# ComputationalPhysiology/oasisx

Hardware: AMD Instinct MI355X
Metric: time-steps/sec, 3D Taylor-Green 128^3 P2-P1 (with pressure-CG SpMV GB/s in roofline) (higher is better)
Workload: dtype f64

## Files before the change

### include/oasisx_hip.h

```cpp
#ifndef OASISX_HIP_H
#define OASISX_HIP_H

#include <stddef.h>
#include <stdint.h>

#ifdef __cplusplus
extern "C" {
#endif

#define OX_KV 2
#define OX_ROW_BLOCK_WAVES 8
#define OX_ROW_BLOCK_LDS (134 * 1024)
#define OX_SLICE 64

#define OX_CONVERGED_RTOL 2
#define OX_CONVERGED_ATOL 3
#define OX_CONVERGED_ITS 4
#define OX_DIVERGED_ITS (-3)
#define OX_DIVERGED_DTOL (-4)
#define OX_DIVERGED_BREAKDOWN (-5)
#define OX_DIVERGED_NANORINF (-9)

#define OX_KSP_CG 1
#define OX_KSP_BCGS 2
// ... 143 lines not shown
int ox_rect_view(const ox_rect *rect, ox_rect_info *view);
int ox_rect_destroy(ox_rect *rect);
int ox_value_dictionary(const double *vals, int64_t n_slots, int ncomp, void *codes, double *dict, int *n_dict,
                        void *stream);
int ox_pair_stream_size(const ox_sell *A, const int32_t *row_len, int64_t *ps_ptr, int64_t *n_codes, void *stream);
int ox_window_retile(const ox_sell *A, const int64_t *wt_ptr, const void *src, int elem_bytes, void *dst, void *stream);
int ox_pair_stream_fill(const ox_sell *A, const int32_t *row_len, int64_t *ps_ptr, uint32_t *ps_code,
                        int32_t *ps_base, int64_t *n_wide, void *stream);
int ox_malloc(size_t bytes, void **out);
int ox_free(void *p);
int ox_memset(void *p, int value, size_t bytes, void *stream);
int ox_synchronize(void *stream);

int ox_version(void);
const char *ox_last_error(void);
int ox_sell_kv(void);
int ox_device_info(int *n_cu, char *name, int name_len);

int ox_spmv(const ox_sell *A, const double *x, double *y, int ncomp, const ox_dist *dist,
            void *stream);

int ox_sell_compress_cols(const ox_sell *A, uint16_t *cols16, int32_t *cbase, int64_t *n_compressed,
                          void *stream);

int ox_spmv_multi(int v2s, int gdim, const ox_sell *A, const double *x, const double *base, double scale,
                  double *y, const ox_dist *dist, void *stream);
int ox_assemble_rect(int family, int row_degree, int col_degree, const ox_cells *cells, const ox_adj *adj,
                     const uint8_t *adj_pos, int pw, const ox_sell *A, void *stream);

int ox_axpby(int64_t n, double a, const double *x, double b, const double *y, double *z,
             void *stream);
int ox_dot(int64_t n_rows, int ncomp, const double *x, const double *y, double *out_host,
           const ox_dist *dist, void *stream);

int ox_set_bc(double *b, const int32_t *dofs, const double *g, int64_t n, int ncomp, int comp,
              void *stream);

int ox_scatter_add(double *b, const int32_t *rows, const double *y, int64_t n, int ncomp, int comp,
                   double scale, void *stream);

int ox_zero_rows(const ox_sell *A, const int32_t *rows, int64_t n, double diag, void *stream);
int ox_zero_rows_au(const ox_sell *A, const int32_t *rows, int64_t n, double diag, double *au,
                    const double *u1, int ncomp, void *stream);
int ox_zero_rows_cols(const ox_sell *A, const uint8_t *is_bc, double diag, void *stream);

int ox_assemble_matrix(int kind, int degree, const ox_cells *cells, const int32_t *cell_dofs,
                       const ox_adj *adj, const uint8_t *adj_pos, int pw, const ox_sell *A,
                       int n_bins, const int64_t *bin_ptr_host, const int32_t *bin_slices,
                       const int32_t *bin_width_host, void *stream);
int ox_assemble_weights(int degree, const ox_cells *cells, const ox_adj *adj, int64_t n_rows,
                        double *w, void *stream);
int ox_assemble_load_vector(const ox_cells *cells, const ox_adj *adj, int64_t n_rows, int n_d, int n_q,
                            const double *wphi, const double *fq, double *b, void *stream);

int ox_assemble_first(int degree, const ox_cells *cells, const int32_t *cell_dofs,
                      const ox_adj *adj, const uint8_t *adj_pos, int pw, const ox_sell *A,
                      const ox_sell *M, const ox_sell *K, const double *uab,
                      const double *u1, const double *b0, double *b_first, double dt, double nu,
                      int n_bins, const int64_t *bin_ptr_host, const int32_t *bin_slices,
                      const int32_t *bin_width_host, void *stream);

int ox_assemble_first_au(int degree, const ox_cells *cells, const int32_t *cell_dofs,
                         const ox_adj *adj, const uint8_t *adj_pos, int pw, const ox_sell *A,
                         const ox_sell *M, const ox_sell *K, const double *uab,
                         const double *u1, const double *b0, double *b_first, double dt, double nu,
                         int n_bins, const int64_t *bin_ptr_host, const int32_t *bin_slices,
// ... 154 lines not shown
```

### oasisx_amd/_lib.py

```python
from __future__ import annotations

import ctypes as C
import os

_HERE = os.path.dirname(os.path.abspath(__file__))
LIB_PATH = os.environ.get("OX_LIB_PATH") or os.path.join(_HERE, "liboasisx_hip.so")

KSP_CG, KSP_BCGS, KSP_CG_SINGLE, KSP_BCGS_MERGED, KSP_CG_MERGED = 1, 2, 3, 4, 5
KSP_CG_MG = 6
MG_MAX_DEGREE = 8
ROW_BLOCK_WAVES, ROW_BLOCK_LDS = 8, 134 * 1024
CONVERGED_RTOL, CONVERGED_ATOL, CONVERGED_ITS = 2, 3, 4
DIVERGED_ITS, DIVERGED_DTOL, DIVERGED_BREAKDOWN, DIVERGED_NANORINF = -3, -4, -5, -9


class OasisxHipError(RuntimeError):
    pass


class ox_sell(C.Structure):
    _fields_ = [
        ("n_rows", C.c_int64),
        ("n_cols", C.c_int64),
        ("n_slices", C.c_int32),
# ... 175 lines not shown

SIGNATURES = {
    "ox_version": (_I, []),
    "ox_last_error": (C.c_char_p, []),
    "ox_sell_kv": (_I, []),
    "ox_device_info": (_I, [C.POINTER(_I), C.c_char_p, _I]),
    "ox_mesh_create": (_I, [_P, _L, _P, _L, _I, _I, _I, C.POINTER(_P)]),
    "ox_mesh_view": (_I, [_P, C.POINTER(ox_mesh_info)]),
    "ox_mesh_destroy": (_I, [_P]),
    "ox_space_create": (_I, [_P, _I, _I, C.POINTER(_P)]),
    "ox_space_create_ordered": (_I, [_P, _I, _I, _I, C.POINTER(_P)]),
    "ox_mesh_create_sub": (_I, [_P, _L, _P, _L, _I, _I, C.POINTER(_D), C.POINTER(_D), _I, _I, _L, C.POINTER(_P)]),
    "ox_space_create_part": (_I, [_P, _I, _I, _P, _L, _I, _L, C.POINTER(_P)]),
    "ox_space_view": (_I, [_P, C.POINTER(ox_space_info)]),
    "ox_space_windows": (_I, [_P, C.POINTER(ox_window_info)]),
    "ox_space_windows_split": (_I, [_P, _I, C.POINTER(ox_window_info)]),
    "ox_space_destroy": (_I, [_P]),
    "ox_rect_create": (_I, [_P, _P, C.POINTER(_P)]),
    "ox_rect_view": (_I, [_P, C.POINTER(ox_rect_info)]),
    "ox_rect_destroy": (_I, [_P]),
    "ox_value_dictionary": (_I, [_P, _L, _I, _P, _P, C.POINTER(_I), _P]),
    "ox_pair_stream_size": (_I, [C.POINTER(ox_sell), _P, _P, C.POINTER(_L), _P]),
    "ox_pair_stream_fill": (_I, [C.POINTER(ox_sell), _P, _P, _P, _P, C.POINTER(_L), _P]),
    "ox_malloc": (_I, [C.c_size_t, C.POINTER(_P)]),
    "ox_free": (_I, [_P]),
    "ox_memset": (_I, [_P, _I, C.c_size_t, _P]),
    "ox_synchronize": (_I, [_P]),
    "ox_spmv": (_I, [C.POINTER(ox_sell), _P, _P, _I, _P, _P]),
    "ox_sell_compress_cols": (_I, [C.POINTER(ox_sell), _P, _P, C.POINTER(_L), _P]),
    "ox_spmv_multi": (_I, [_I, _I, C.POINTER(ox_sell), _P, _P, _D, _P, _P, _P]),
    "ox_assemble_rect": (_I, [_I, _I, _I, C.POINTER(ox_cells), C.POINTER(ox_adj), _P, _I, C.POINTER(ox_sell), _P]),
    "ox_axpby": (_I, [_L, _D, _P, _D, _P, _P, _P]),
    "ox_dot": (_I, [_L, _I, _P, _P, C.POINTER(_D), _P, _P]),
    "ox_set_bc": (_I, [_P, _P, _P, _L, _I, _I, _P]),
    "ox_scatter_add": (_I, [_P, _P, _P, _L, _I, _I, _D, _P]),
    "ox_zero_rows": (_I, [C.POINTER(ox_sell), _P, _L, _D, _P]),
    "ox_zero_rows_au": (_I, [C.POINTER(ox_sell), _P, _L, _D, _P, _P, _I, _P]),
    "ox_zero_rows_cols": (_I, [C.POINTER(ox_sell), _P, _D, _P]),
    "ox_assemble_matrix": (_I, [_I, _I, C.POINTER(ox_cells), _P, C.POINTER(ox_adj), _P, _I,
                                C.POINTER(ox_sell), _I, C.POINTER(_L), _P, C.POINTER(C.c_int32), _P]),
    "ox_assemble_weights": (_I, [_I, C.POINTER(ox_cells), C.POINTER(ox_adj), _L, _P, _P]),
    "ox_assemble_load_vector": (_I, [C.POINTER(ox_cells), C.POINTER(ox_adj), _L, _I, _I, _P, _P, _P, _P]),
    "ox_assemble_first": (_I, [_I, C.POINTER(ox_cells), _P, C.POINTER(ox_adj), _P, _I,
                               C.POINTER(ox_sell), C.POINTER(ox_sell), C.POINTER(ox_sell), _P, _P, _P, _P, _D,
                               _D, _I, C.POINTER(_L), _P, C.POINTER(C.c_int32), _P]),
    "ox_assemble_first_au": (_I, [_I, C.POINTER(ox_cells), _P, C.POINTER(ox_adj), _P, _I,
                                  C.POINTER(ox_sell), C.POINTER(ox_sell), C.POINTER(ox_sell), _P, _P, _P, _P, _D,
                                  _D, _I, C.POINTER(_L), _P, C.POINTER(C.c_int32), _P, _P]),
    "ox_assemble_matrix_blocks": (_I, [_I, _I, C.POINTER(ox_cells), _P, C.POINTER(ox_adj), _P, _I, C.POINTER(ox_sell), _I, _P,
                                       _L, _P]),
    "ox_assemble_first_blocks": (_I, [_I, C.POINTER(ox_cells), _P, C.POINTER(ox_adj), _P, _I,
                                      C.POINTER(ox_sell), C.POINTER(ox_sell), C.POINTER(ox_sell), _P, _P, _P, _P, _D,
                                      _D, _I, _P, _L, _P, _P]),
    "ox_assemble_grad_vector": (_I, [_I, _I, _I, C.POINTER(ox_cells), _P, C.POINTER(ox_adj), _L, _P,
                                     _P, _D, _P, _P]),
    "ox_assemble_div_vector": (_I, [_I, _I, C.POINTER(ox_cells), _P, C.POINTER(ox_adj), _L, _P, _D,
                                    _P, _P]),
    "ox_dg1_grad_rhs": (_I, [_I, C.POINTER(ox_cells), _P, _P, _P, _P]),
    "ox_dg1_mass": (_I, [_I, C.POINTER(ox_cells), _I, _P, _P, _P]),
    "ox_jacobi_setup": (_I, [C.POINTER(ox_sell), _P, _P]),
    "ox_ksp_work_bytes": (C.c_size_t, [_L, _L, _I, _I]),
    "ox_ksp_solve": (_I, [_I, C.POINTER(ox_sell), _P, _P, _P, _I, _D, _D, _I, _I, _I, _I, _P,
                          C.c_size_t, C.POINTER(ox_ksp_result), _P, _P]),
    "ox_ksp_solve_ax0": (_I, [_I, C.POINTER(ox_sell), _P, _P, _P, _I, _D, _D, _I, _I, _I, _I, _P,
                              C.c_size_t, C.POINTER(ox_ksp_result), _P, _P, _P]),
    "ox_ksp_solve_dc": (_I, [_I, C.POINTER(ox_sell), _P, _P, _P, _I, _D, _D, _I, _I, _I, _I, _P,
# ... 102 lines not shown
```

### oasisx_amd/csrc/ox_ksp.hip

```cpp
#include "ox_kernels.h"
#include "ox_ksp_dev.h"
#include "ox_p2p.h"
#include <type_traits>

struct KspPart2 {
  const double *partial;
  int nparts, nv;
};

__device__ __forceinline__ void ksp_gather2(const double *__restrict__ partial, int nparts, int nv, const KspPart2 &B,
                                            double (&v)[OX_MAX_NV]) {
  ox_gather_partials(partial, nparts, nv, v);
  if (B.nv > 0) {
    double w[OX_MAX_NV];
    ox_gather_partials(B.partial, B.nparts, B.nv, w);
#pragma unroll
    for (int i = 0; i < OX_MAX_NV; ++i)
#pragma unroll
      for (int j = 0; j < OX_MAX_NV; ++j)
        if (j == i - nv && j < B.nv) v[i] = w[j];
  }
}


// ... 654 lines not shown
    }
  });
  ksp_store_partial<2 * NC>(s, red, partial);
}

template <int NC>
__global__ __launch_bounds__(256) void k_bcgs_init(int64_t n, const double *__restrict__ b,
                                                   double *x, const double *q,
                                                   const double *__restrict__ dinv, double *vr,
                                                   double *vrhat, double *vp, double *vv, int guess,
                                                   double *partial) {
  __shared__ double red[4 * 2 * NC];
  double s[2 * NC];
#pragma unroll
  for (int i = 0; i < 2 * NC; ++i) s[i] = 0.0;
  ox_flat_pairs<NC>(n, [&](int64_t e, int ca, int64_t ra, int cb, int64_t rb, bool two) {
    const double2 bb = ox_ld2(b, e, two);
    double2 r = bb;
    if (guess) {
      const double2 qq = ox_ld2(q, e, two);
      r.x -= qq.x;
      r.y -= qq.y;
    } else {
      double2 z;
      z.x = z.y = 0.0;
      ox_st2(x, e, z, two);
    }
    const double d0 = dinv[ra], d1 = two ? dinv[rb] : 0.0;
    r.x *= d0;
    r.y *= d1;
    const double db0 = d0 * bb.x, db1 = d1 * bb.y;
    ox_st2(vr, e, r, two);
    ox_st2(vrhat, e, r, two);
    ox_st2(vp, e, r, two);
    ox_acc<NC>(s, 0, ca, r.x, r.x);
    ox_acc<NC>(s, NC, ca, db0, db0);
    if (two) {
      ox_acc<NC>(s, 0, cb, r.y, r.y);
      ox_acc<NC>(s, NC, cb, db1, db1);
    }
  });
  ksp_store_partial<2 * NC>(s, red, partial);
}

template <int NC>
__global__ __launch_bounds__(256) void k_bcgs_p(int64_t n, const KspState *S, int c0,
                                                const double *__restrict__ vr, double *vp,
                                                const double *__restrict__ vv, double *vrhat) {
  if (S->done) return;
  double beta[NC], omega[NC], reseed[NC];
  bool any = false;
#pragma unroll
  for (int c = 0; c < NC; ++c) {
    beta[c] = S->beta[c0 + c];
    omega[c] = S->omega[c0 + c];
    reseed[c] = S->restart[c0 + c] ? 1.0 : 0.0;
    any = any || S->restart[c0 + c];
  }
  ox_flat_pairs<NC>(n, [&](int64_t e, int ca, int64_t, int cb, int64_t, bool two) {
    const double2 r = ox_ld2(vr, e, two), v = ox_ld2(vv, e, two);
    double2 p = ox_ld2(vp, e, two);
    const bool ra = ox_sel<NC>(reseed, ca) != 0.0, rb = ox_sel<NC>(reseed, cb) != 0.0;
    p.x = ra ? r.x : fma(ox_sel<NC>(beta, ca), fma(-ox_sel<NC>(omega, ca), v.x, p.x), r.x);
    p.y = rb ? r.y : fma(ox_sel<NC>(beta, cb), fma(-ox_sel<NC>(omega, cb), v.y, p.y), r.y);
    ox_st2(vp, e, p, two);
    if (any) {
      double2 h = ox_ld2(vrhat, e, two);
      h.x = ra ? r.x : h.x;
      h.y = rb ? r.y : h.y;
      ox_st2(vrhat, e, h, two);
    }
  });
}

template <int NC>
__global__ __launch_bounds__(256) void k_bcgs_s(int64_t n, const KspState *S, int c0,
                                                const double *__restrict__ vr,
                                                const double *__restrict__ vv, double *vs) {
  if (S->done) return;
  double alpha[NC];
#pragma unroll
  for (int c = 0; c < NC; ++c) alpha[c] = S->alpha[c0 + c];
  ox_flat_pairs<NC>(n, [&](int64_t e, int ca, int64_t, int cb, int64_t, bool two) {
    const double2 r = ox_ld2(vr, e, two), v = ox_ld2(vv, e, two);
    double2 s;
    s.x = fma(-ox_sel<NC>(alpha, ca), v.x, r.x);
    s.y = fma(-ox_sel<NC>(alpha, cb), v.y, r.y);
    ox_st2(vs, e, s, two);
  });
}

template <int NC>
__global__ __launch_bounds__(256) void k_bcgs_x(int64_t n, const KspState *S, int c0, double *x, double *vr,
                                                const double *__restrict__ vrhat,
// ... 165 lines not shown
    if (B.nv > 0 && (int64_t)B.nparts * B.nv >= OX_PRERED_MIN) {
      const int g = ksp_prered_rows(B.nparts);
      hipLaunchKernelGGL(k_prereduce, dim3(g), dim3(256), 0, st, B.partial, B.nparts, B.nv, scr);
      B.partial = scr;
      B.nparts = g;
    }
  }
  const int nmax = nparts > B.nparts ? nparts : B.nparts;
  if (!dist) {
    hipLaunchKernelGGL((k_ksp_scalar<PH>), dim3(1), dim3(ox_red_threads(nmax)), 0, st, S, partial, nparts, nv, P, B);
    OX_LAUNCH_CHECK();
    return 0;
  }
  if (ox_prof_on) ox_prof_start(OX_TAG_SYNC_POINT, st, nv + B.nv);
  if (dist->p2p && dist->nranks <= 64) {
    int threads = ox_red_threads(nmax);
    if (threads < ox_p2p_ar_threads(dist->nranks)) threads = ox_p2p_ar_threads(dist->nranks);
    hipLaunchKernelGGL((k_ksp_scalar_p2p<PH>), dim3(1), dim3(threads), 0, st, S, partial, nparts, nv, P,
                       ox_p2p_next_allreduce(dist), B);
    if (ox_prof_on) ox_prof_stop(st);
    OX_LAUNCH_CHECK();
    return 0;
  }
  hipLaunchKernelGGL((k_ksp_reduce<PH>), dim3(1), dim3(ox_red_threads(nmax)), 0, st, partial, nparts, nv, B, sums);
  OX_LAUNCH_CHECK();
  nv += B.nv;
  if (ox_allreduce_impl(dist, sums, nv, st)) return -1;
  hipLaunchKernelGGL((k_ksp_logic<PH>), dim3(1), dim3(64), 0, st, S, sums, P);
  if (ox_prof_on) ox_prof_stop(st);
  OX_LAUNCH_CHECK();
  return 0;
}

__global__ __launch_bounds__(256) void k_extract_col(int64_t n, const double *__restrict__ src, int nc,
                                                     int c, double *__restrict__ dst) {
  const int64_t stride = (int64_t)gridDim.x * 256;
  for (int64_t i = (int64_t)blockIdx.x * 256 + threadIdx.x; i < n; i += stride) dst[i] = src[i * nc + c];
}
__global__ __launch_bounds__(256) void k_insert_col(int64_t n, const double *__restrict__ src, int nc,
                                                    int c, double *__restrict__ dst) {
  const int64_t stride = (int64_t)gridDim.x * 256;
  for (int64_t i = (int64_t)blockIdx.x * 256 + threadIdx.x; i < n; i += stride) dst[i * nc + c] = src[i];
}

struct KspVecs {
  double *x, *r, *z, *p, *q;
  double *rhat, *v, *s, *t;
  double *u, *w;
};

struct KspCtx {
  const ox_sell *A;
  const double *dinv;
  KspDinv D;
  KspState *S, *S2;
  double *sums, *partial, *partial2;
  const ox_dist *dist;
  hipStream_t st;
  int nb, nbs;
  int fold;
};

#define KSP_SYNC(PH, partial, nparts, nv)                                                       \
  do {                                                                                          \
    if (ksp_sync_point<PH>(C.S, partial, nparts, nv, C.sums, P, C.dist, C.st)) return -1;       \
  } while (0)

static int ksp_fold_blocks_default() {
  static int dflt = -1;
  if (dflt < 0) {
// ... 239 lines not shown
  for (int k = 0; k < count; ++k) {
    ox_spmv_set_epilogue_dinv(C.D.code, C.D.dict);
    const int rc = ox_spmv_dist(C.A, V.p, V.q, NC, OX_EPI_CG_M2, C.dinv, nullptr, C.partial, done, C.dist, C.st);
    ox_spmv_set_epilogue_dinv(nullptr, nullptr);
    if (rc) return -1;
    KspParams Q = ksp_last_point(P, k, count);
    Q.first = (first && k == 0) ? 1 : 0;
    if (ksp_sync_point<PH_CGM_IT>(C.S, C.partial, C.nbs, 2 * NC, C.sums, Q, C.dist, C.st,
                                  Q.first ? KspPart2{nullptr, 0, 0} : KspPart2{C.partial2, C.nb, 3 * NC}))
      return -1;
    hipLaunchKernelGGL((k_cgm_update<NC>), dim3(C.nb), dim3(256), 0, C.st, n, C.S, P.c0, V.x, V.r, V.q, C.D, V.p, C.partial2);
    OX_LAUNCH_CHECK();
  }
  return 0;
}

template <int NC>
static int cgs_iterations(const KspCtx &C, const KspVecs &V, const KspParams &P, int count) {
  const int64_t n = C.A->n_rows;
  const int *done = &C.S->done;
  for (int k = 0; k < count; ++k) {
    hipLaunchKernelGGL((k_cgs_update<NC>), dim3(C.nb), dim3(256), 0, C.st, n, C.S, P.c0, V.x, V.r, V.u, V.p, V.s, V.w,
                       C.dinv, C.partial);
    OX_LAUNCH_CHECK();
    if (ox_spmv_dist(C.A, V.u, V.w, NC, OX_EPI_DOT, nullptr, nullptr, C.partial2, done, C.dist, C.st)) return -1;
    if (ksp_sync_point<PH_CGS_IT>(C.S, C.partial, C.nb, 2 * NC, C.sums, ksp_last_point(P, k, count), C.dist, C.st,
                                  KspPart2{C.partial2, C.nbs, NC}))
      return -1;
  }
  return 0;
}

template <int NC>
static int bcgs_iterations(const KspCtx &C, const KspVecs &V, const KspParams &P, int count, bool first) {
  const int64_t n = C.A->n_rows;
  const int *done = &C.S->done;
  for (int k = 0; k < count; ++k) {
    if (!(first && k == 0)) {
      hipLaunchKernelGGL((k_bcgs_p<NC>), dim3(C.nb), dim3(256), 0, C.st, n, C.S, P.c0, V.r, V.p, V.v, V.rhat);
      OX_LAUNCH_CHECK();
    }
    if (ox_spmv_dist(C.A, V.p, V.v, NC, OX_EPI_BCGS_V, C.dinv, V.rhat, C.partial, done, C.dist, C.st)) return -1;
    KSP_SYNC(PH_BCGS_1, C.partial, C.nbs, NC);
    hipLaunchKernelGGL((k_bcgs_s<NC>), dim3(C.nb), dim3(256), 0, C.st, n, C.S, P.c0, V.r, V.v, V.s);
    OX_LAUNCH_CHECK();
    if (ox_spmv_dist(C.A, V.s, V.t, NC, OX_EPI_BCGS_T, C.dinv, nullptr, C.partial, done, C.dist, C.st)) return -1;
    KSP_SYNC(PH_BCGS_2, C.partial, C.nbs, 2 * NC);
    hipLaunchKernelGGL((k_bcgs_x<NC>), dim3(C.nb), dim3(256), 0, C.st, n, C.S, P.c0, V.x, V.r, V.rhat, V.p, V.s,
                       V.t, C.partial, 0);
    OX_LAUNCH_CHECK();
    if (ksp_sync_point<PH_BCGS_3>(C.S, C.partial, C.nb, 2 * NC, C.sums, ksp_last_point(P, k, count), C.dist, C.st)) return -1;
  }
  return 0;
}

template <int NC>
static int bcgsm_iterations(const KspCtx &C, const KspVecs &V, const KspParams &P, int count, bool first) {
  const int64_t n = C.A->n_rows;
  const int *done = &C.S->done;
  (void)first;
  for (int k = 0; k < count; ++k) {
    if (ox_spmv_dist(C.A, V.p, V.v, NC, OX_EPI_BCGS_V, C.dinv, V.rhat, C.partial, done, C.dist, C.st)) return -1;
    if (ksp_sync_point<PH_BCGS_1>(C.S, C.partial, C.nbs, NC, C.sums, P, C.dist, C.st)) return -1;
    hipLaunchKernelGGL((k_bcgs_s<NC>), dim3(C.nb), dim3(256), 0, C.st, n, C.S, P.c0, V.r, V.v, V.s);
    OX_LAUNCH_CHECK();
    if (ox_spmv_dist(C.A, V.s, V.t, NC, OX_EPI_BCGS_T5, C.dinv, V.rhat, C.partial, done, C.dist, C.st)) return -1;
    if (ksp_sync_point<PH_BCGSM_B>(C.S, C.partial, C.nbs, 5 * NC, C.sums, ksp_last_point(P, k, count), C.dist, C.st)) return -1;
    hipLaunchKernelGGL((k_bcgs_xp<NC>), dim3(C.nb), dim3(256), 0, C.st, n, C.S, P.c0, V.x, V.r, V.rhat, V.p, V.s, V.t, V.v, 0);
    OX_LAUNCH_CHECK();
  }
  return 0;
}
template <int NC>
static int bcgsm_finish(const KspCtx &C, const KspVecs &V, const KspParams &P) {
  hipLaunchKernelGGL((k_bcgs_xp<NC>), dim3(C.nb), dim3(256), 0, C.st, C.A->n_rows, C.S, P.c0, V.x, V.r, V.rhat, V.p, V.s, V.t,
                     V.v, 1);
  OX_LAUNCH_CHECK();
  return 0;
}

static int ksp_read_state(const KspCtx &C) {
  OX_HIP(hipMemcpyAsync(g_state_host, C.S, sizeof(KspState), hipMemcpyDeviceToHost, C.st));
  OX_HIP(hipStreamSynchronize(C.st));
  return C.dist ? ox_dist_status(C.dist) : 0;
// ... 62 lines not shown
  double *vec[6];
  for (int i = 0; i < L.nvec; ++i) vec[i] = reinterpret_cast<double *>(work + L.vec0 + L.vec_stride * i);
  if (!g_state_host) OX_HIP(hipHostMalloc(&g_state_host, 3 * sizeof(KspState)));
  const bool cg = ksp_type == OX_KSP_CG, cgs = ksp_type == OX_KSP_CG_SINGLE, bm = ksp_type == OX_KSP_BCGS_MERGED;
  const bool cgm = ksp_type == OX_KSP_CG_MERGED;
  KspVecs V{};
  V.x = x;
  if (cgs) {
    V.r = vec[0], V.u = vec[1], V.p = vec[2], V.s = vec[3], V.w = vec[4];
    if (guess && !ax0) {
      if (ox_spmv_dist(A, x, V.w, NC, OX_EPI_NONE, nullptr, nullptr, nullptr, nullptr, dist, st)) return -1;
    }
    hipLaunchKernelGGL((k_cgs_init<NC>), dim3(C.nb), dim3(256), 0, st, n, b, x, (guess && ax0) ? ax0 : V.w, dinv, V.r, V.u,
                       V.p, V.s, guess, C.partial);
    OX_LAUNCH_CHECK();
    if (ox_spmv_dist(A, V.u, V.w, NC, OX_EPI_DOT, nullptr, nullptr, C.partial2, nullptr, dist, st)) return -1;
    if (ksp_sync_point<PH_CGS_INIT>(C.S, C.partial, C.nb, 3 * NC, C.sums, P, dist, st, KspPart2{C.partial2, C.nbs, NC}))
      return -1;
  } else if (cg || cgm) {
    V.r = vec[0], V.p = vec[1], V.q = vec[2];
    if (guess && !ax0) {
      if (ox_spmv_dist(A, x, V.q, NC, OX_EPI_NONE, nullptr, nullptr, nullptr, nullptr, dist, st)) return -1;
    }
    hipLaunchKernelGGL((k_cg_init<NC>), dim3(C.nb), dim3(256), 0, st, n, b, x, (guess && ax0) ? ax0 : V.q, dinv, V.r,
                       V.p, guess, C.partial);
    OX_LAUNCH_CHECK();
    KSP_SYNC(PH_CG_INIT, C.partial, C.nb, 3 * NC);
  } else {
    V.r = vec[0], V.rhat = vec[1], V.p = vec[2], V.v = vec[3], V.s = vec[4], V.t = vec[5];
    if (guess && !ax0) {
      if (ox_spmv_dist(A, x, V.t, NC, OX_EPI_NONE, nullptr, nullptr, nullptr, nullptr, dist, st)) return -1;
    }
    hipLaunchKernelGGL((k_bcgs_init<NC>), dim3(C.nb), dim3(256), 0, st, n, b, x, (guess && ax0) ? ax0 : V.t, dinv, V.r,
                       V.rhat, V.p, V.v, guess, C.partial);
    OX_LAUNCH_CHECK();
    KSP_SYNC(PH_BCGS_INIT, C.partial, C.nb, 2 * NC);
  }
  bool bm_first = true;
  auto iterate = [&](auto nc_tag, const KspVecs &W, const KspParams &Q) -> int {
    constexpr int N_ = decltype(nc_tag)::value;
    const bool first = bm_first;
    bm_first = false;
    return cgs ? cgs_iterations<N_>(C, W, Q, check_every)
           : cgm ? cgm_iterations<N_>(C, W, Q, check_every, first)
               : (cg ? cg_iterations<N_>(C, W, Q, check_every)
                     : (bm ? bcgsm_iterations<N_>(C, W, Q, check_every, first) : bcgs_iterations<N_>(C, W, Q, check_every, first)));
  };
  auto batch_of = [&](int every) { return every > 8 ? 8 : every; };
  int it = 0;
  bool tail_done = false;
  for (;;) {
    tail_done = false;
    if (NC == 1 && run_ahead) {
      const int bsz = batch_of(check_every);
      auto it1 = [&](int count) -> int {
        const bool first = bm_first;
        bm_first = false;
        return cgs ? cgs_iterations<1>(C, V, P, count)
               : cgm ? cgm_iterations<1>(C, V, P, count, first)
                   : (cg ? cg_iterations<1>(C, V, P, count)
                         : (bm ? bcgsm_iterations<1>(C, V, P, count, first) : bcgs_iterations<1>(C, V, P, count, first)));
      };
      if (ksp_run_ahead(C, it1, bsz, it, P.max_it)) return -1;
    }
    for (; !(NC == 1 && run_ahead) && it <= P.max_it; it += check_every) {
      if (iterate(std::integral_constant<int, NC>{}, V, P)) return -1;
      if (ksp_read_state(C)) return -1;
      if (g_state_host->done) break;
      if (NC > 1) {
        int live = -1, nlive = 0;
        for (int c = 0; c < NC; ++c)
          if (g_state_host->active[c]) live = c, ++nlive;
        if (nlive == 1) {
          double *cv[8];
          for (int i = 0; i < 8; ++i) cv[i] = reinterpret_cast<double *>(work + L.narrow0 + L.narrow_stride * i);
          KspVecs W{};
          double *src[8] = {V.x, V.r, V.z, V.p, V.q, V.rhat, V.v, nullptr};
          double **dst[8] = {&W.x, &W.r, &W.z, &W.p, &W.q, &W.rhat, &W.v, nullptr};
          if (cg) src[2] = nullptr;
          if (cgs) {
            src[2] = V.u, dst[2] = &W.u;
            src[4] = V.s, dst[4] = &W.s;
            src[5] = V.w, dst[5] = &W.w;
            src[6] = nullptr;
          }
          for (int i = 0; i < 7; ++i) {
            *dst[i] = cv[i];
            if (!src[i]) continue;
            hipLaunchKernelGGL(k_extract_col, dim3(C.nb), dim3(256), 0, st, n, src[i], NC, live, cv[i]);
            OX_LAUNCH_CHECK();
          }
          if (!cgs) {
            W.s = cv[2];
            W.t = cv[4];
          }
          KspParams P1 = P;
          P1.nc = 1;
          P1.c0 = live;
          if (run_ahead) {
            const int bsz = batch_of(check_every);
            auto it1 = [&](int count) -> int {
              return cgs ? cgs_iterations<1>(C, W, P1, count)
                         : (cg ? cg_iterations<1>(C, W, P1, count)
                               : (bm ? bcgsm_iterations<1>(C, W, P1, count, false) : bcgs_iterations<1>(C, W, P1, count, false)));
            };
            it += check_every;
            if (ksp_run_ahead(C, it1, bsz, it, P.max_it)) return -1;
          } else {
            for (it += check_every; it <= P.max_it; it += check_every) {
              if (iterate(std::integral_constant<int, 1>{}, W, P1)) return -1;
              if (ksp_read_state(C)) return -1;
              if (g_state_host->done) break;
            }
          }
          if (cg) {
            hipLaunchKernelGGL((k_cg_update2<1>), dim3(C.nb), dim3(256), 0, st, n, C.S, P1.c0, W.x, W.r, C.D, W.p, 1);
            OX_LAUNCH_CHECK();
          }
          if (bm && g_state_host->its[live] > 0) {
            if (bcgsm_finish<1>(C, W, P1)) return -1;
            hipLaunchKernelGGL(k_insert_col, dim3(C.nb), dim3(256), 0, st, n, W.r, NC, live, V.r);
            OX_LAUNCH_CHECK();
          }
          tail_done = true;
          hipLaunchKernelGGL(k_insert_col, dim3(C.nb), dim3(256), 0, st, n, W.x, NC, live, x);
          OX_LAUNCH_CHECK();
          break;
        }
      }
    }
    if (!g_state_host->done) OX_FAIL("ox_ksp_solve: device state never reported completion");
    if (!bm) break;
    bool any = false;
    for (int c = 0; c < NC; ++c) any = any || g_state_host->its[c] > 0;
    if (!any) break;
    if (!tail_done && bcgsm_finish<NC>(C, V, P)) return -1;
    bool retest = false;
    for (int c = 0; c < NC; ++c)
      retest = retest || g_state_host->reason[c] == OX_CONVERGED_RTOL || g_state_host->reason[c] == OX_CONVERGED_ATOL;
    if (!retest) break;
    hipLaunchKernelGGL((k_rr<NC>), dim3(C.nb), dim3(256), 0, st, n, V.r, C.partial);
    OX_LAUNCH_CHECK();
    KSP_SYNC(PH_BCGSM_FIN, C.partial, C.nb, NC);
    if (ksp_read_state(C)) return -1;
    if (g_state_host->done) break;
    hipLaunchKernelGGL((k_bcgs_p<NC>), dim3(C.nb), dim3(256), 0, st, n, C.S, P.c0, V.r, V.p, V.v, V.rhat);
    OX_LAUNCH_CHECK();
    it = 0;
    for (int c = 0; c < NC; ++c) it = g_state_host->its[c] > it ? g_state_host->its[c] : it;
  }
  if (cg && !tail_done) {
    hipLaunchKernelGGL((k_cg_update2<NC>), dim3(C.nb), dim3(256), 0, st, n, C.S, P.c0, V.x, V.r, C.D, V.p, 1);
    OX_LAUNCH_CHECK();
  }
  for (int c = 0; c < NC; ++c) {
    result->reason[c] = g_state_host->reason[c];
    result->its[c] = g_state_host->its[c];
    result->rnorm[c] = g_state_host->rn[c];
    result->bnorm[c] = g_state_host->bn[c];
    result->resumed[c] = bm ? g_state_host->nresume[c] : 0;
  }
  return 0;
}

__global__ __launch_bounds__(256) void k_mgcg_init(int64_t n, const double *__restrict__ b, double *x,
                                                   const double *__restrict__ q, double *r, int guess) {
  OX_ROW_LOOP {
    if (guess) {
      r[row] = b[row] - q[row];
    } else {
      r[row] = b[row];
      x[row] = 0.0;
    }
  }
}
template <bool INIT>
__global__ __launch_bounds__(256) void k_mgcg_dots(int64_t n, const KspState *S, const double *__restrict__ r,
                                                   const double *__restrict__ z, const double *__restrict__ zb, double *p,
                                                   double *partial) {
// ... 211 lines not shown
                               size_t work_bytes, ox_ksp_result *result, const ox_dist *dist, void *stream,
                               const double *ax0, const uint8_t *dinv_code, const double *dinv_dict, int n_dinv_dict) {
  ox_ksp_options o;
  ox_ksp_options_default(&o);
  o.rtol = rtol;
  o.atol = atol;
  o.max_it = max_it;
  o.nonzero_guess = nonzero_guess;
  o.check_every = check_every;
  o.max_restarts = max_restarts;
  o.ax0 = ax0;
  o.dinv_code = dinv_code;
  o.dinv_dict = dinv_dict;
  o.n_dinv_dict = n_dinv_dict;
  return ox_ksp_solve_opt(ksp_type, A, dinv, b, x, ncomp, &o, work, work_bytes, result, dist, stream);
}

extern "C" int ox_ksp_solve_ax0(int ksp_type, const ox_sell *A, const double *dinv, const double *b,
                                double *x, int ncomp, double rtol, double atol, int max_it,
                                int nonzero_guess, int check_every, int max_restarts, void *work,
                                size_t work_bytes, ox_ksp_result *result, const ox_dist *dist, void *stream,
                                const double *ax0) {
  return ox_ksp_solve_dc(ksp_type, A, dinv, b, x, ncomp, rtol, atol, max_it, nonzero_guess, check_every, max_restarts,
                         work, work_bytes, result, dist, stream, ax0, nullptr, nullptr, 0);
}

extern "C" int ox_ksp_solve(int ksp_type, const ox_sell *A, const double *dinv, const double *b,
                            double *x, int ncomp, double rtol, double atol, int max_it,
                            int nonzero_guess, int check_every, int max_restarts, void *work,
                            size_t work_bytes, ox_ksp_result *result, const ox_dist *dist, void *stream) {
  return ox_ksp_solve_dc(ksp_type, A, dinv, b, x, ncomp, rtol, atol, max_it, nonzero_guess, check_every, max_restarts,
                         work, work_bytes, result, dist, stream, nullptr, nullptr, nullptr, 0);
}
```

### oasisx_amd/fracstep.py

```python
from __future__ import annotations

import ctypes as C
import logging

import numpy as np
import torch

from . import _lib
from .fem import FieldStorage, Function, FunctionSpace, VectorFunctionSpace, cell_geometry
from .ksp import KSPSolver
from .la import MultiSellMatrix, SellMatrix

__all__ = ["FractionalStep_AB_CN"]


def _degree(element):
    if isinstance(element, FunctionSpace):
        return element.degree
    fam = str(element[0]).lower()
    if fam not in ("lagrange", "p", "cg"):
        raise ValueError(f"unsupported element family {element[0]!r}")
    return int(element[1])


# ... 303 lines not shown
        if self._scalar_groups:
            self._A_pre_bc = True
            try:
                self.scalar_assemble(dt, nu)
            finally:
                self._A_pre_bc = False
        for bcp in self._bcs_p:
            bcp.update_bc()
            bcp.add_surface_terms(self._BFIRST)
        for bcu in self._bcs_u[0]:
            self._A.zero_rows(bcu._rows_dev, 1.0, self._B3.ptr() if want_au else None,
                              self._U1.rptr() if want_au else None, self._gdim)
        self._AU1_valid = want_au

    @_phase
    def velocity_tentative_assemble(self):
        Vi, Q = self._Vi[0][0], self._Q
        if not self._low_memory:
            self._p_vdxi_Mat.mult(False, self._PS.ptr(), self._BFIRST.ptr(), 1.0, self._RHS1.ptr())
            return
        _lib.check(self._lib.ox_assemble_grad_vector(0, Vi.degree, Q.degree, C.byref(self._cells),
                                                     _lib.ptr(Q.cell_dofs), C.byref(self._adj_u), Vi.n_owned,
                                                     self._PS.ptr(), self._BFIRST.ptr(), 1.0, self._RHS1.ptr(),
                                                     _lib.current_stream()), "ox_assemble_grad_vector")

    @_phase
    def velocity_tentative_solve(self):
        lib, st = self._lib, _lib.current_stream()
        gdim = self._gdim
        for i in range(gdim):
            for bc in self._bcs_u[i]:
                bc.apply(self._rhs1[i].x)
        n = self._n_u * gdim
        _lib.check(lib.ox_axpby(n, 1.0, self._U.rptr(), 0.0, None, self._WRK.ptr(), st), "ox_axpby")
        ax0 = None
        if getattr(self, "_AU1_valid", False):
            self._AU1_valid = False
            same = getattr(self, "_u_is_u1", None) == (self._U.generation, self._U1.generation)
            if self._part is not None and getattr(self._comm, "size", 1) > 1:
                same = self._comm.allreduce(0.0 if same else 1.0, op="max") == 0.0
            if same:
                ax0 = self._B3
            elif not getattr(self, "_shortcut_note", False):
                self._shortcut_note = True
                logging.getLogger("oasisx").info(
                    "tentative solve: u was handed out writable since the last step (FieldStorage.dev() / ptr() / host()): "
                    "the A u1 product of assemble_first is not reused; read-only access goes through rdev() / rptr() / rhost()")
        self._u_is_u1 = None
        errors = np.asarray(self._solver_u.solve_block(self._RHS1, self._U, ax0=ax0), dtype=np.int32)
        _lib.check(lib.ox_axpby(n, 1.0, self._WRK.ptr(), -1.0, self._U.ptr(), self._WRK.ptr(), st), "ox_axpby")
        out = (C.c_double * 4)()
        _lib.check(lib.ox_dot(self._no_u, gdim, self._WRK.ptr(), self._WRK.ptr(), out, self._du, st), "ox_dot")
        diff = float(sum(np.sqrt(out[i]) for i in range(gdim)))
        return diff, errors

    @_phase
    def pressure_assemble(self, dt: float):
        Vi, Q = self._Vi[0][0], self._Q
        if not self._low_memory:
            self._divu_Mat.mult(True, self._U.ptr(), None, -1.0 / float(dt), self._B2.ptr())
        else:
            _lib.check(self._lib.ox_assemble_div_vector(Q.degree, Vi.degree, C.byref(self._cells),
                                                        _lib.ptr(Vi.cell_dofs), C.byref(self._adj_q), Q.n_owned,
                                                        self._U.ptr(), -1.0 / float(dt), self._B2.ptr(),
                                                        _lib.current_stream()), "ox_assemble_div_vector")
        for bcp in self._bcs_p:
            bcp.apply_homogeneous(self._b2.x)

    @_phase
    def pressure_solve(self, nu: float | None = None, rotational: bool = False):
        lib, st = self._lib, _lib.current_stream()
        logger = logging.getLogger("oasisx")
        nq, nqo = self._n_q, self._no_q
        if len(self._bcs_p) == 0:
            if "ksp_error_if_not_converged" not in self._solver_p._options:
                self._solver_p.updateOptions({"ksp_error_if_not_converged": 1})
            _lib.check(lib.ox_remove_mean(nqo, nqo, self._B2.ptr(), None, float(self._Q.num_dofs_global),
                                          self._dq, st), "ox_remove_mean")
        converged = self._solver_p.solve_block(self._B2, self._DP)[0]
        if len(self._bcs_p) == 0:
            logger.debug("Making sure that mean of phi is 0 with lack of pressure conditions")
            _lib.check(lib.ox_remove_mean(nqo, nq, self._DP.ptr(), _lib.ptr(self._wQ), self._vol, self._dq, st),
                       "ox_remove_mean")
        if self._projector_p is not None:
            if nu is None:
# ... 104 lines not shown
```

Before: 12.22.

## Fuse velocity diff norm, skip redundant copies in BiCGStab and column extraction

Replaces the copy-then-axpby-then-dot sequence in the tentative velocity solve with a fused difference-norm kernel, and skips the initial copy of u entirely when u still equals u1. In BiCGStab the first-iteration search direction is read from rhat instead of writing a separate p vector, using a small state machine. The per-vector column extraction launches are batched into a single kernel. The aim is to cut memory traffic and launch count, at the cost of more complex state tracking for p across the batched and split paths.

```diff
diff --git a/include/oasisx_hip.h b/include/oasisx_hip.h
--- a/include/oasisx_hip.h
+++ b/include/oasisx_hip.h
@@ -199,6 +199,8 @@
              void *stream);
 int ox_dot(int64_t n_rows, int ncomp, const double *x, const double *y, double *out_host,
            const ox_dist *dist, void *stream);
+int ox_diff_norm2(int64_t n_rows, int ncomp, const double *x, const double *y, double *out_host,
+                  const ox_dist *dist, void *stream);
 
 int ox_set_bc(double *b, const int32_t *dofs, const double *g, int64_t n, int ncomp, int comp,
               void *stream);
diff --git a/oasisx_amd/_lib.py b/oasisx_amd/_lib.py
--- a/oasisx_amd/_lib.py
+++ b/oasisx_amd/_lib.py
@@ -231,6 +231,7 @@
     "ox_assemble_rect": (_I, [_I, _I, _I, C.POINTER(ox_cells), C.POINTER(ox_adj), _P, _I, C.POINTER(ox_sell), _P]),
     "ox_axpby": (_I, [_L, _D, _P, _D, _P, _P, _P]),
     "ox_dot": (_I, [_L, _I, _P, _P, C.POINTER(_D), _P, _P]),
+    "ox_diff_norm2": (_I, [_L, _I, _P, _P, C.POINTER(_D), _P, _P]),
     "ox_set_bc": (_I, [_P, _P, _P, _L, _I, _I, _P]),
     "ox_scatter_add": (_I, [_P, _P, _P, _L, _I, _I, _D, _P]),
     "ox_zero_rows": (_I, [C.POINTER(ox_sell), _P, _L, _D, _P]),
diff --git a/oasisx_amd/csrc/ox_ksp.hip b/oasisx_amd/csrc/ox_ksp.hip
--- a/oasisx_amd/csrc/ox_ksp.hip
+++ b/oasisx_amd/csrc/ox_ksp.hip
@@ -710,7 +710,7 @@
     const double db0 = d0 * bb.x, db1 = d1 * bb.y;
     ox_st2(vr, e, r, two);
     ox_st2(vrhat, e, r, two);
-    ox_st2(vp, e, r, two);
+    if (vp) ox_st2(vp, e, r, two);
     ox_acc<NC>(s, 0, ca, r.x, r.x);
     ox_acc<NC>(s, NC, ca, db0, db0);
     if (two) {
@@ -724,7 +724,7 @@
 template <int NC>
 __global__ __launch_bounds__(256) void k_bcgs_p(int64_t n, const KspState *S, int c0,
                                                 const double *__restrict__ vr, double *vp,
-                                                const double *__restrict__ vv, double *vrhat) {
+                                                const double *__restrict__ vv, double *vrhat, const double *vpin) {
   if (S->done) return;
   double beta[NC], omega[NC], reseed[NC];
   bool any = false;
@@ -737,7 +737,7 @@
   }
   ox_flat_pairs<NC>(n, [&](int64_t e, int ca, int64_t, int cb, int64_t, bool two) {
     const double2 r = ox_ld2(vr, e, two), v = ox_ld2(vv, e, two);
-    double2 p = ox_ld2(vp, e, two);
+    double2 p = ox_ld2(vpin, e, two);
     const bool ra = ox_sel<NC>(reseed, ca) != 0.0, rb = ox_sel<NC>(reseed, cb) != 0.0;
     p.x = ra ? r.x : fma(ox_sel<NC>(beta, ca), fma(-ox_sel<NC>(omega, ca), v.x, p.x), r.x);
     p.y = rb ? r.y : fma(ox_sel<NC>(beta, cb), fma(-ox_sel<NC>(omega, cb), v.y, p.y), r.y);
@@ -969,10 +969,22 @@
   return 0;
 }
 
-__global__ __launch_bounds__(256) void k_extract_col(int64_t n, const double *__restrict__ src, int nc,
-                                                     int c, double *__restrict__ dst) {
+struct KspExtract {
+  const double *src[6];
+  double *dst[6];
+  int count;
+};
+__global__ __launch_bounds__(256) void k_extract_cols(int64_t n, KspExtract E, int nc, int c) {
   const int64_t stride = (int64_t)gridDim.x * 256;
-  for (int64_t i = (int64_t)blockIdx.x * 256 + threadIdx.x; i < n; i += stride) dst[i] = src[i * nc + c];
+  for (int64_t i = (int64_t)blockIdx.x * 256 + threadIdx.x; i < n; i += stride) {
+    double v[6];
+#pragma unroll
+    for (int k = 0; k < 6; ++k)
+      if (k < E.count) v[k] = E.src[k][i * nc + c];
+#pragma unroll
+    for (int k = 0; k < 6; ++k)
+      if (k < E.count) E.dst[k][i] = v[k];
+  }
 }
 __global__ __launch_bounds__(256) void k_insert_col(int64_t n, const double *__restrict__ src, int nc,
                                                     int c, double *__restrict__ dst) {
@@ -1278,24 +1290,28 @@
 }
 
 template <int NC>
-static int bcgs_iterations(const KspCtx &C, const KspVecs &V, const KspParams &P, int count, bool first) {
+static int bcgs_iterations(const KspCtx &C, const KspVecs &V, const KspParams &P, int count, int &pstate) {
   const int64_t n = C.A->n_rows;
   const int *done = &C.S->done;
   for (int k = 0; k < count; ++k) {
-    if (!(first && k == 0)) {
-      hipLaunchKernelGGL((k_bcgs_p<NC>), dim3(C.nb), dim3(256), 0, C.st, n, C.S, P.c0, V.r, V.p, V.v, V.rhat);
+    if (pstate == 1 || pstate == 2) {
+      hipLaunchKernelGGL((k_bcgs_p<NC>), dim3(C.nb), dim3(256), 0, C.st, n, C.S, P.c0, V.r, V.p, V.v, V.rhat,
+                         pstate == 1 ? V.rhat : V.p);
       OX_LAUNCH_CHECK();
-    }
-    if (ox_spmv_dist(C.A, V.p, V.v, NC, OX_EPI_BCGS_V, C.dinv, V.rhat, C.partial, done, C.dist, C.st)) return -1;
+      pstate = 2;
+    }
+    const double *p = pstate == 0 ? V.rhat : V.p;
+    if (ox_spmv_dist(C.A, const_cast<double *>(p), V.v, NC, OX_EPI_BCGS_V, C.dinv, V.rhat, C.partial, done, C.dist, C.st)) return -1;
     KSP_SYNC(PH_BCGS_1, C.partial, C.nbs, NC);
     hipLaunchKernelGGL((k_bcgs_s<NC>), dim3(C.nb), dim3(256), 0, C.st, n, C.S, P.c0, V.r, V.v, V.s);
     OX_LAUNCH_CHECK();
     if (ox_spmv_dist(C.A, V.s, V.t, NC, OX_EPI_BCGS_T, C.dinv, nullptr, C.partial, done, C.dist, C.st)) return -1;
     KSP_SYNC(PH_BCGS_2, C.partial, C.nbs, 2 * NC);
-    hipLaunchKernelGGL((k_bcgs_x<NC>), dim3(C.nb), dim3(256), 0, C.st, n, C.S, P.c0, V.x, V.r, V.rhat, V.p, V.s,
+    hipLaunchKernelGGL((k_bcgs_x<NC>), dim3(C.nb), dim3(256), 0, C.st, n, C.S, P.c0, V.x, V.r, V.rhat, p, V.s,
                        V.t, C.partial, 0);
     OX_LAUNCH_CHECK();
     if (ksp_sync_point<PH_BCGS_3>(C.S, C.partial, C.nb, 2 * NC, C.sums, ksp_last_point(P, k, count), C.dist, C.st)) return -1;
+    pstate = pstate == 0 ? 1 : 2;
   }
   return 0;
 }
@@ -1424,11 +1440,12 @@
       if (ox_spmv_dist(A, x, V.t, NC, OX_EPI_NONE, nullptr, nullptr, nullptr, nullptr, dist, st)) return -1;
     }
     hipLaunchKernelGGL((k_bcgs_init<NC>), dim3(C.nb), dim3(256), 0, st, n, b, x, (guess && ax0) ? ax0 : V.t, dinv, V.r,
-                       V.rhat, V.p, V.v, guess, C.partial);
+                       V.rhat, (bm || dist) ? V.p : nullptr, V.v, guess, C.partial);
     OX_LAUNCH_CHECK();
     KSP_SYNC(PH_BCGS_INIT, C.partial, C.nb, 2 * NC);
   }
   bool bm_first = true;
+  int bcgs_p_state = dist ? 3 : 0;
   auto iterate = [&](auto nc_tag, const KspVecs &W, const KspParams &Q) -> int {
     constexpr int N_ = decltype(nc_tag)::value;
     const bool first = bm_first;
@@ -1436,7 +1453,7 @@
     return cgs ? cgs_iterations<N_>(C, W, Q, check_every)
            : cgm ? cgm_iterations<N_>(C, W, Q, check_every, first)
                : (cg ? cg_iterations<N_>(C, W, Q, check_every)
-                     : (bm ? bcgsm_iterations<N_>(C, W, Q, check_every, first) : bcgs_iterations<N_>(C, W, Q, check_every, first)));
+                     : (bm ? bcgsm_iterations<N_>(C, W, Q, check_every, first) : bcgs_iterations<N_>(C, W, Q, check_every, bcgs_p_state)));
   };
   auto batch_of = [&](int every) { return every > 8 ? 8 : every; };
   int it = 0;
@@ -1451,7 +1468,7 @@
         return cgs ? cgs_iterations<1>(C, V, P, count)
                : cgm ? cgm_iterations<1>(C, V, P, count, first)
                    : (cg ? cg_iterations<1>(C, V, P, count)
-                         : (bm ? bcgsm_iterations<1>(C, V, P, count, first) : bcgs_iterations<1>(C, V, P, count, first)));
+                         : (bm ? bcgsm_iterations<1>(C, V, P, count, first) : bcgs_iterations<1>(C, V, P, count, bcgs_p_state)));
       };
       if (ksp_run_ahead(C, it1, bsz, it, P.max_it)) return -1;
     }
@@ -1476,12 +1493,18 @@
             src[5] = V.w, dst[5] = &W.w;
             src[6] = nullptr;
           }
+          if (cg) src[4] = nullptr;
+          if (bcgs_p_state < 2 && !cg && !cgs && !bm) src[3] = V.rhat;
+          KspExtract E{};
           for (int i = 0; i < 7; ++i) {
             *dst[i] = cv[i];
             if (!src[i]) continue;
-            hipLaunchKernelGGL(k_extract_col, dim3(C.nb), dim3(256), 0, st, n, src[i], NC, live, cv[i]);
-            OX_LAUNCH_CHECK();
+            E.src[E.count] = src[i], E.dst[E.count] = cv[i];
+            ++E.count;
           }
+          hipLaunchKernelGGL(k_extract_cols, dim3(C.nb), dim3(256), 0, st, n, E, NC, live);
+          OX_LAUNCH_CHECK();
+          bcgs_p_state = 2;
           if (!cgs) {
             W.s = cv[2];
             W.t = cv[4];
@@ -1494,7 +1517,7 @@
             auto it1 = [&](int count) -> int {
               return cgs ? cgs_iterations<1>(C, W, P1, count)
                          : (cg ? cg_iterations<1>(C, W, P1, count)
-                               : (bm ? bcgsm_iterations<1>(C, W, P1, count, false) : bcgs_iterations<1>(C, W, P1, count, false)));
+                               : (bm ? bcgsm_iterations<1>(C, W, P1, count, false) : bcgs_iterations<1>(C, W, P1, count, bcgs_p_state)));
             };
             it += check_every;
             if (ksp_run_ahead(C, it1, bsz, it, P.max_it)) return -1;
@@ -1536,7 +1559,7 @@
     KSP_SYNC(PH_BCGSM_FIN, C.partial, C.nb, NC);
     if (ksp_read_state(C)) return -1;
     if (g_state_host->done) break;
-    hipLaunchKernelGGL((k_bcgs_p<NC>), dim3(C.nb), dim3(256), 0, st, n, C.S, P.c0, V.r, V.p, V.v, V.rhat);
+    hipLaunchKernelGGL((k_bcgs_p<NC>), dim3(C.nb), dim3(256), 0, st, n, C.S, P.c0, V.r, V.p, V.v, V.rhat, V.p);
     OX_LAUNCH_CHECK();
     it = 0;
     for (int c = 0; c < NC; ++c) it = g_state_host->its[c] > it ? g_state_host->its[c] : it;
@@ -1814,3 +1837,53 @@
   return ox_ksp_solve_dc(ksp_type, A, dinv, b, x, ncomp, rtol, atol, max_it, nonzero_guess, check_every, max_restarts,
                          work, work_bytes, result, dist, stream, nullptr, nullptr, nullptr, 0);
 }
+
+template <int NC>
+__global__ __launch_bounds__(256) void k_diff_norm2(int64_t n_rows, const double *__restrict__ x, const double *__restrict__ y,
+                                                    double *__restrict__ partial) {
+  __shared__ double red[4 * NC];
+  double s[NC];
+#pragma unroll
+  for (int c = 0; c < NC; ++c) s[c] = 0.0;
+  const int64_t stride = (int64_t)gridDim.x * 256;
+  for (int64_t r = (int64_t)blockIdx.x * 256 + threadIdx.x; r < n_rows; r += stride) {
+#pragma unroll
+    for (int c = 0; c < NC; ++c) {
+      const double d = x[r * NC + c] - y[r * NC + c];
+      s[c] = fma(d, d, s[c]);
+    }
+  }
+  ox_block_sum_256<NC>(s, red);
+  if (threadIdx.x == 0) {
+#pragma unroll
+    for (int c = 0; c < NC; ++c) partial[(size_t)blockIdx.x * NC + c] = s[c];
+  }
+}
+
+static thread_local double *g_diff_scratch = nullptr;
+static thread_local double *g_diff_scratch_host = nullptr;
+
+extern "C" int ox_diff_norm2(int64_t n_rows, int ncomp, const double *x, const double *y, double *out_host,
+                             const ox_dist *dist, void *stream) {
+  if (ncomp < 1 || ncomp > OX_MAXC) OX_FAIL("ox_diff_norm2: ncomp=%d", ncomp);
+  if (!x || !y || !out_host) OX_FAIL("ox_diff_norm2: null argument");
+  if (!g_diff_scratch) {
+    OX_HIP(hipMalloc(&g_diff_scratch, sizeof(double) * (OX_VEC_MAX_BLOCKS * 4 + 16)));
+    OX_HIP(hipHostMalloc(&g_diff_scratch_host, sizeof(double) * 16));
+  }
+  hipStream_t st = ox_stream(stream);
+  const int nblk = ox_vec_blocks(n_rows > 0 ? n_rows : 1);
+  double *partial = g_diff_scratch, *sums = g_diff_scratch + OX_VEC_MAX_BLOCKS * 4;
+  switch (ncomp) {
+    case 1: hipLaunchKernelGGL(k_diff_norm2<1>, dim3(nblk), dim3(256), 0, st, n_rows, x, y, partial); break;
+    case 2: hipLaunchKernelGGL(k_diff_norm2<2>, dim3(nblk), dim3(256), 0, st, n_rows, x, y, partial); break;
+    default: hipLaunchKernelGGL(k_diff_norm2<3>, dim3(nblk), dim3(256), 0, st, n_rows, x, y, partial); break;
+  }
+  OX_LAUNCH_CHECK();
+  if (ox_reduce_partials(partial, nblk, ncomp, sums, st)) return -1;
+  if (dist && ox_allreduce_impl(dist, sums, ncomp, st)) return -1;
+  OX_HIP(hipMemcpyAsync(g_diff_scratch_host, sums, sizeof(double) * ncomp, hipMemcpyDeviceToHost, st));
+  OX_HIP(hipStreamSynchronize(st));
+  for (int c = 0; c < ncomp; ++c) out_host[c] = g_diff_scratch_host[c];
+  return 0;
+}
diff --git a/oasisx_amd/fracstep.py b/oasisx_amd/fracstep.py
--- a/oasisx_amd/fracstep.py
+++ b/oasisx_amd/fracstep.py
@@ -359,11 +359,14 @@
             for bc in self._bcs_u[i]:
                 bc.apply(self._rhs1[i].x)
         n = self._n_u * gdim
-        _lib.check(lib.ox_axpby(n, 1.0, self._U.rptr(), 0.0, None, self._WRK.ptr(), st), "ox_axpby")
+        self._U.rptr(), self._U1.rptr()
+        old_is_u1 = getattr(self, "_u_is_u1", None) == (self._U.generation, self._U1.generation)
+        if not old_is_u1:
+            _lib.check(lib.ox_axpby(n, 1.0, self._U.rptr(), 0.0, None, self._WRK.ptr(), st), "ox_axpby")
         ax0 = None
         if getattr(self, "_AU1_valid", False):
             self._AU1_valid = False
-            same = getattr(self, "_u_is_u1", None) == (self._U.generation, self._U1.generation)
+            same = old_is_u1
             if self._part is not None and getattr(self._comm, "size", 1) > 1:
                 same = self._comm.allreduce(0.0 if same else 1.0, op="max") == 0.0
             if same:
@@ -375,9 +378,9 @@
                     "the A u1 product of assemble_first is not reused; read-only access goes through rdev() / rptr() / rhost()")
         self._u_is_u1 = None
         errors = np.asarray(self._solver_u.solve_block(self._RHS1, self._U, ax0=ax0), dtype=np.int32)
-        _lib.check(lib.ox_axpby(n, 1.0, self._WRK.ptr(), -1.0, self._U.ptr(), self._WRK.ptr(), st), "ox_axpby")
         out = (C.c_double * 4)()
-        _lib.check(lib.ox_dot(self._no_u, gdim, self._WRK.ptr(), self._WRK.ptr(), out, self._du, st), "ox_dot")
+        u_old = self._U1.rptr() if old_is_u1 else self._WRK.rptr()
+        _lib.check(lib.ox_diff_norm2(self._no_u, gdim, u_old, self._U.rptr(), out, self._du, st), "ox_diff_norm2")
         diff = float(sum(np.sqrt(out[i]) for i in range(gdim)))
         return diff, errors
 
```

Measured after the change: 12.33 (median of 6 runs). Within noise of the previous version (+0.9%).
